# Jan-Celin/SCCG-genome-compression

Measured on AMD Instinct MI355X. Metric: target bases compressed/sec at 1/2/4/8 GPUs; bit-exact record stream vs CPU ref, higher is better.
Workload: dtype u8

## Files before the change

sccg-genome-compression_amd/csrc/walk.hip:

```cpp
#include "internal.h"

#include <algorithm>
#include <chrono>
#include <map>
#include <mutex>
#include <cstdio>
#include <cstdlib>
#include <vector>

namespace {

constexpr int WPB = 4;
constexpr int WWPB = 4;
constexpr int WCAP = 256;
constexpr int32_t INVALID = INT32_MIN;
constexpr int32_t NEVER = INT32_MIN + 1;
constexpr int ANCHOR_K = 32;
constexpr int KEY_K = 15;
constexpr int KMAX = 32;
constexpr int KB_COUNT = 32;
constexpr int ANCHOR_STEP = 64;
constexpr int ANCHOR_LOAD = 1;
constexpr int ANCHOR_PROBE_BATCHES = 2;
constexpr uint32_t A_MULTI = 0xFFFFFFFFu;
constexpr int ANCHOR_RETRIES = 8;
constexpr int32_t ANCHOR_RETRY_STEP = 512;
constexpr int32_t FROZEN_MIN = 4096;
constexpr int FROZEN_MAX = 256;
constexpr int FROZEN_FIRST = 16;

enum ChunkKind : int32_t { KIND_SPEC = 0, KIND_FIX = 1, KIND_RESUME = 2 };
enum ChunkStatus : int32_t { ST_OK = 0, ST_ESC = 1, ST_CONV = 3, ST_DONE = 4 };
constexpr int32_t RESEED_GAP = 1024;
constexpr int32_t TRAP_P = 4096;
constexpr int RESPEC_AHEAD = 256;
constexpr int RESPEC_MAX_TRIGGERS = 64;
constexpr int32_t LONG_GAP = 4096;
constexpr int32_t CAND_CAP = 65536;
constexpr int CH_BAND = 512;
constexpr int CH_TBITS = CH_BAND <= 2048 ? 13 : 14;
constexpr int CH_GRID = 512;
constexpr int CH_HCAP = 4096;
constexpr int32_t CHAIN_MCAP = 1 << 22;
constexpr int CH_GENS_PER_SYNC = 4;
constexpr int FF_MIN_CHUNKS = 8;
constexpr int64_t CH_FF_SPAN = 32 * 1024;
constexpr int CH_MAX_GENS = 4096;
constexpr int MARCH_ROUNDS = 4;
constexpr int CHAIN_ROUND = 10;
constexpr int64_t CH_DENSE_HITS = 32768;
constexpr int CH_DENSE_N = 32;
constexpr int32_t CH_DENSE_SPAN = 8192;
constexpr int CH_HANDBACK_N = 64;

struct WalkPtrs {
    const uint8_t* R;
    const uint8_t* T;
    int32_t nR, nT, k, m, S, C, cap;
    int32_t kp;
    int32_t xlo, xhi;
    int32_t* bt[2];
    int32_t* bp[2];
    int32_t* bl[2];
    int32_t* cnt[2];
    int32_t* cur;
    int32_t* exitX;
    int32_t* exitP;
    int32_t* usedX;
    int32_t* usedP;
    int32_t* kind;
    int32_t* status;
    int32_t* escX;
    int32_t* escP;
    int32_t* escN;
    int32_t* escQ;
    int32_t* snapX;
    int32_t* snapP;
    int32_t* guess;
    int32_t* plist;
    int32_t* rlist;
    int32_t* clist;
    int32_t* newX;
    int32_t* newP;
    int32_t* conv;
    int32_t* changed;
    int32_t* walked;
    int32_t* lround;
    int32_t* seedq;
    int32_t* trapped;
    int32_t* frozen;
    int32_t* flist;
    int32_t* fy;
    int32_t* scal;
    int32_t* trig;
    int32_t* tflag;
    int32_t* fa_j;
    int32_t* fa_l;
    int32_t* fa_p;
    int32_t* hintY;
    int32_t* hintP;
    uint64_t* atab;
    uint32_t agen;
    int32_t adet;
    uint32_t* fbits;
    uint32_t* cbits;
    int32_t round;
    int32_t abits;
    const int64_t* dnR;
    int32_t astep;
    unsigned long long* fc;
    unsigned long long* fcb;
    int32_t* cand;
    uint8_t* kb;
    int64_t* flat_off;
    int32_t* ft;
    int32_t* fp;
    int32_t* fl;
    int64_t* tlen;
    int64_t* partial;
    int64_t* scal64;
    int64_t* lgap;
    int64_t* cprev;
    int64_t* ctext;
    int64_t lgap_cap;
    int32_t* chs;
    int32_t* chm_t;
    int32_t* chm_p;
    int32_t* chm_l;
    int32_t chm_cap;
    int32_t ch_settled;
    int32_t* chh_y;
    uint32_t* chh_k;
    int32_t* chh_n;
    int32_t* chh_tr;
    uint64_t* dbg;
    int32_t dbg_phases;
    int32_t dbg_round;
};

__device__ __forceinline__ int32_t chunk_lo(const WalkPtrs& A, int32_t j) { return A.xlo + j * A.S; }
__device__ __forceinline__ int32_t chunk_hi(const WalkPtrs& A, int32_t j) {
    const int32_t lo = A.xlo + j * A.S;
    return lo + A.S < A.xhi ? lo + A.S : A.xhi;
}

constexpr int WFBITS = 14;
constexpr int LBV = 2048;
constexpr int LBW = LBV / 256;
static_assert(LBW % 8 == 0, "whole 32-byte stretches per lane");
constexpr int LEAD = 128;
static_assert(LEAD % (4 * LBW) == 0, "the lead is whole lanes' stretches");
__device__ __forceinline__ uint32_t wf_h1(uint32_t key) { return slot_hash(key, WFBITS); }
__device__ __forceinline__ uint32_t wf_h2(uint32_t key) { return (key * 0x85EBCA77u) >> (32 - WFBITS); }
__device__ __forceinline__ uint32_t wf_h3(uint32_t key) { return (key * 0xC2B2AE3Du + 0x27D4EB2Fu) >> (32 - WFBITS); }
struct WalkLds {
    uint32_t wbits[1 << (WFBITS - 5)];
    __attribute__((aligned(16))) uint8_t rbuf[LBV + 64];
    __attribute__((aligned(16))) uint8_t tbuf[LBV + 64];
};
constexpr int32_t NO_BUF = INT32_MIN / 2;
struct BufPos {
    int32_t rb0 = NO_BUF, tb0 = NO_BUF;
    __device__ __forceinline__ bool has_r(int32_t a, int32_t n) const { return a >= rb0 && a + n <= rb0 + LBV; }
    __device__ __forceinline__ bool has_t(int32_t a, int32_t n) const { return a >= tb0 && a + n <= tb0 + LBV; }
};

__device__ __forceinline__ uint64_t pick_key(int32_t p, int32_t pme) {
    const int32_t d = p - pme;
    return ((uint64_t)(uint32_t)(d < 0 ? -d : d) << 32) | (uint32_t)p;
}

__device__ __forceinline__ bool bytes_eq(const uint8_t* a, const uint8_t* b, int k) {
    for (int i = 0; i < k; i++) if (a[i] != b[i]) return false;
    return true;
}

template <int ND>
__device__ __forceinline__ void loadw_lds(const uint8_t* lds, int32_t off, uint32_t (&o)[ND]) {
    const uint32_t* w = reinterpret_cast<const uint32_t*>(lds) + (off >> 2);
    const uint32_t sh = (uint32_t)(off & 3);
    uint32_t v[ND + 1];
#pragma unroll
    for (int i = 0; i <= ND; i++) v[i] = w[i];
#pragma unroll
    for (int i = 0; i < ND; i++) o[i] = __builtin_amdgcn_alignbyte(v[i + 1], v[i], sh);
}

template <int ND>
__device__ __forceinline__ void loadw_sel(bool in_lds, const uint8_t* lds, int32_t lds_off, const uint8_t* g,
                                          uint32_t (&o)[ND]) {
    if (in_lds) {
        loadw_lds<ND>(lds, lds_off, o);
    } else {
        loadw<ND>(g, o);
        asm volatile("" ::: "memory");
    }
}

template <int N>
__device__ __forceinline__ int first_diff(const uint32_t (&r)[N], const uint32_t (&t)[N]) {
    int pos = 4 * N;
#pragma unroll
    for (int i = N - 1; i >= 0; i--) {
        const uint32_t x = r[i] ^ t[i];
        if (x) pos = 4 * i + (__builtin_ctz(x) >> 3);
    }
    return pos;
}
__device__ __forceinline__ int first_diff32(const uint32_t (&r)[8], const uint32_t (&t)[8]) { return first_diff<8>(r, t); }

__device__ __forceinline__ void lds16(const uint8_t* lds, int32_t off, uint32_t (&o)[4]) {
    const int32_t a = off + 16 * lane_id();
    const uint2* p = reinterpret_cast<const uint2*>(lds + (a & ~7));
    const uint2 v0 = p[0], v1 = p[1], v2 = p[2];
    const uint32_t sh = (uint32_t)(off & 3);
    uint32_t w[5];
    if (off & 4) { w[0] = v0.y; w[1] = v1.x; w[2] = v1.y; w[3] = v2.x; w[4] = v2.y; }
    else { w[0] = v0.x; w[1] = v0.y; w[2] = v1.x; w[3] = v1.y; w[4] = v2.x; }
#pragma unroll
    for (int i = 0; i < 4; i++) o[i] = __builtin_amdgcn_alignbyte(w[i + 1], w[i], sh);
}

__device__ __forceinline__ int32_t lds_first_diff(const uint8_t* rbuf, int32_t ra, const uint8_t* tbuf, int32_t tb, int32_t n) {
    const int lane = lane_id();
    for (int32_t base = 0; base < n; base += 1024) {
        const int32_t lim = n - base - 16 * lane;
        int e = 16;
        if (lim > 0) {
            uint32_t r[4], t[4];
            lds16(rbuf, ra + base, r);
            lds16(tbuf, tb + base, t);
            e = first_diff<4>(r, t);
            if (e >= lim) e = 16;
        }
        const unsigned long long m = __ballot(e < 16);
        if (m) {
            const int l = first_lane(m);
            return base + 16 * l + lane_val(e, l);
        }
    }
    return n;
}

__device__ __forceinline__ int32_t wave_lce(const WalkPtrs& A, WalkLds& L, BufPos& B, int32_t a, int32_t b, int32_t maxlen) {
    const int lane = lane_id();
    if (maxlen <= 0) return 0;
    int32_t off = 0;
    if (a >= B.rb0 && b >= B.tb0 && a < B.rb0 + LBV && b < B.tb0 + LBV) {
        int32_t avail = B.rb0 + LBV - a < B.tb0 + LBV - b ? B.rb0 + LBV - a : B.tb0 + LBV - b;
        if (avail > maxlen) avail = maxlen;
        const int32_t e = lds_first_diff(L.rbuf, a - B.rb0, L.tbuf, b - B.tb0, avail);
        if (e < avail || avail >= maxlen) return e;
        off = avail;
    }
    while (off < maxlen) {
        const int32_t lead = (a + off >= LEAD && b + off >= LEAD) ? LEAD : 0;
        const int32_t sa = (a + off - lead) & ~15, sb = (b + off - lead) & ~15;
        static_assert(LBV == 2048, "two KiB of each per step");
        const uint4* gr = reinterpret_cast<const uint4*>(A.R + sa) + lane;
        const uint4* gt = reinterpret_cast<const uint4*>(A.T + sb) + lane;
        const uint4 r0 = gr[0], r1 = gr[64], t0 = gt[0], t1 = gt[64];
        wave_sync();
        {
            uint4* dr = reinterpret_cast<uint4*>(L.rbuf) + lane;
            uint4* dt = reinterpret_cast<uint4*>(L.tbuf) + lane;
            dr[0] = r0; dr[64] = r1;
            dt[0] = t0; dt[64] = t1;
        }
        wave_sync();
        B.rb0 = sa;
        B.tb0 = sb;
        const int32_t ra = a + off - sa, tb = b + off - sb;
        int32_t avail = LBV - (ra > tb ? ra : tb);
        if (avail > maxlen - off) avail = maxlen - off;
        const int32_t e = lds_first_diff(L.rbuf, ra, L.tbuf, tb, avail);
        if (e < avail) return off + e;
        off += avail;
    }
    return maxlen;
}


__device__ int32_t wave_lce_hbm(const uint8_t* __restrict__ R, int32_t a, const uint8_t* __restrict__ T, int32_t b,
                                int32_t maxlen) {
    const int lane = lane_id();
    for (int32_t off = 0; off < maxlen; off += 2048) {
        const int32_t my = off + 32 * lane;
        int32_t e = INT32_MAX;
        if (maxlen - my > 0) {
            uint32_t r[8], t[8];
            loadw<8>(R + a + my, r);
            loadw<8>(T + b + my, t);
            int pos = first_diff32(r, t);
            if (maxlen - my < 32 && pos > maxlen - my) pos = maxlen - my;
            if (pos < 32) e = my + pos;
        }
        const unsigned long long sm = __ballot(e != INT32_MAX);
        if (sm) {
            const int32_t m = lane_val(e, first_lane(sm));
            return m < maxlen ? m : maxlen;
        }
    }
    return maxlen > 0 ? maxlen : 0;
}

__device__ __forceinline__ int32_t ext_k(const WalkPtrs& A, WalkLds& L, BufPos& B, int32_t c, int32_t y) {
    const int32_t kp = A.kp;
    int32_t maxlen = A.nR - (c + kp);
    const int32_t mt = A.nT - (y + kp);
    if (mt < maxlen) maxlen = mt;
    const int32_t l = kp + wave_lce(A, L, B, c + kp, y + kp, maxlen);
    return l >= A.k ? l : 0;
}

constexpr uint32_t KEY_NONE = 0x40000000u;
struct RegWin {
    int32_t P, lo, n;
    uint32_t key[4];
    uint32_t vmask;
};

__device__ __forceinline__ void reg_window(const WalkPtrs& A, int32_t P, RegWin& W, const WalkLds* L = nullptr,
                                           const BufPos* B = nullptr) {
    const int lane = lane_id(), k = A.k;
    W.P = P;
    W.lo = P - A.m < 0 ? 0 : P - A.m;
    const int32_t hi = (P + A.m < A.nR - k) ? P + A.m : A.nR - k;
    W.n = hi - W.lo + 1;
    if (W.n < 0) W.n = 0;
    W.vmask = 0;
    W.key[0] = W.key[1] = W.key[2] = W.key[3] = KEY_NONE;
    const bool lds = L && B->has_r(W.lo, W.n + 20);
    const int i0 = 4 * lane;
    if (i0 >= W.n) return;
    uint32_t w[5];
    loadw_sel<5>(lds, lds ? L->rbuf : nullptr, lds ? W.lo - B->rb0 + i0 : 0, A.R + W.lo + i0, w);
    uint64_t code;
    uint32_t bad;
    pack_codes<5>(w, code, bad);
    const int kp = A.kp;
    const uint32_t MASK = (1u << (2 * kp)) - 1u, KM = (1u << kp) - 1u;
#pragma unroll
    for (int q = 0; q < 4; q++) {
        W.key[q] = (bad >> q) & KM ? exotic_key(A.R + W.lo + i0 + q, kp) : (uint32_t)(code >> (2 * q)) & MASK;
        if (i0 + q < W.n) W.vmask |= 1u << q;
        else W.key[q] = KEY_NONE;
    }
}

__device__ __forceinline__ uint32_t target_key_w(const WalkPtrs& A, int32_t y, const uint32_t (&w)[4]) {
    const int kp = A.kp;
    uint64_t code;
    uint32_t bad;
    pack_codes<4>(w, code, bad);
    return bad & ((1u << kp) - 1u) ? exotic_key(A.T + y, kp) : (uint32_t)code & ((1u << (2 * kp)) - 1u);
}

__device__ __forceinline__ uint32_t win_match(const WalkPtrs& A, const RegWin& W, uint32_t kk, int32_t y) {
    uint32_t m = 0;
#pragma unroll
    for (int q = 0; q < 4; q++)
        if (((W.vmask >> q) & 1u) && W.key[q] == kk) m |= 1u << q;
    if (m && kk >= KEY_EXOTIC) {
        const int32_t c0 = W.lo + 4 * lane_id();
        for (int q = 0; q < 4; q++)
            if (((m >> q) & 1u) && !bytes_eq(A.R + c0 + q, A.T + y, A.kp)) m &= ~(1u << q);
    }
    return m;
}

__device__ __forceinline__ bool win_any(const RegWin& W, uint32_t kk) {
    return (W.key[0] == kk) | (W.key[1] == kk) | (W.key[2] == kk) | (W.key[3] == kk);
}

__device__ void bloom_window(const RegWin& W, WalkLds& L) {
    const int lane = lane_id();
    uint4* b4 = reinterpret_cast<uint4*>(L.wbits);
    for (int i = lane; i < (1 << (WFBITS - 5)) / 4; i += 64) b4[i] = make_uint4(0, 0, 0, 0);
    wave_sync();
#pragma unroll
    for (int q = 0; q < 4; q++) {
        if ((W.vmask >> q) & 1u) {
            const uint32_t f1 = wf_h1(W.key[q]), f2 = wf_h2(W.key[q]), f3 = wf_h3(W.key[q]);
            atomicOr(&L.wbits[f1 >> 5], 1u << (f1 & 31));
            atomicOr(&L.wbits[f2 >> 5], 1u << (f2 & 31));
            atomicOr(&L.wbits[f3 >> 5], 1u << (f3 & 31));
        }
    }
    wave_sync();
}

constexpr int WIDE = 16;
constexpr int WIDE_DEPTH = 1;
__device__ __forceinline__ int32_t wide_step(const WalkPtrs& A, const WalkLds& L, const RegWin& W, int32_t base, int32_t end,
                                             const uint32_t (&w)[8]) {
    const int lane = lane_id(), k = A.kp;
    const uint32_t MASK = (1u << (2 * k)) - 1u, KM = (1u << k) - 1u;
    const int32_t p0 = base + WIDE * lane;
    uint64_t code;
    uint32_t bad;
    pack_codes<8>(w, code, bad);
    uint32_t cand = 0;
#pragma unroll
    for (int st = 0; st < WIDE; st++) {
        const uint32_t key = (bad >> st) & KM ? KEY_EXOTIC : (uint32_t)(code >> (2 * st)) & MASK;
        const uint32_t f1 = wf_h1(key), f2 = wf_h2(key), f3 = wf_h3(key);
        if (key == KEY_EXOTIC ||
            ((L.wbits[f1 >> 5] >> (f1 & 31)) & (L.wbits[f2 >> 5] >> (f2 & 31)) & (L.wbits[f3 >> 5] >> (f3 & 31)) & 1u))
            cand |= 1u << st;
    }
    const int32_t lim = end - p0;
    if (lim < WIDE) cand &= lim > 0 ? (1u << lim) - 1u : 0u;
    for (unsigned long long hm = __ballot(cand != 0); hm; hm &= hm - 1) {
        const int l = __ffsll((long long)hm) - 1;
        uint32_t c = lane_val(cand, l);
        const uint32_t clo = lane_val((uint32_t)code, l), chi = lane_val((uint32_t)(code >> 32), l);
        const uint32_t cbad = lane_val(bad, l);
        const uint64_t lc = ((uint64_t)chi << 32) | clo;
        while (c) {
            const int st = __ffs((int)c) - 1;
            c &= c - 1;
            const int32_t y = base + WIDE * l + st;
            const uint32_t key = (cbad >> st) & KM ? exotic_key(A.T + y, k) : (uint32_t)(lc >> (2 * st)) & MASK;
            if (__ballot(win_match(A, W, key, y) != 0)) return y;
        }
    }
    return -1;
}

__device__ __forceinline__ int32_t wide_scan(const WalkPtrs& A, const WalkLds& L, const RegWin& W, int32_t x, int32_t end) {
    const int lane = lane_id();
    uint32_t w[WIDE_DEPTH][8];
#pragma unroll
    for (int d = 0; d < WIDE_DEPTH; d++)
        if (x + 64 * WIDE * d < end) loadw<8>(A.T + x + 64 * WIDE * d + WIDE * lane, w[d]);
    for (int32_t base = x; base < end;) {
#pragma unroll
        for (int d = 0; d < WIDE_DEPTH; d++) {
            uint32_t cur[8];
#pragma unroll
            for (int i = 0; i < 8; i++) cur[i] = w[d][i];
            const int32_t nb = base + 64 * WIDE * WIDE_DEPTH;
            if (nb < end) loadw<8>(A.T + nb + WIDE * lane, w[d]);
            const int32_t y = wide_step(A, L, W, base, end, cur);
            if (y >= 0) return y;
            base += 64 * WIDE;
            if (base >= end) return end;
        }
    }
    return end;
}

__device__ int32_t anchor_diag(const WalkPtrs& A, int32_t y0);
__device__ __forceinline__ int32_t anchor_diag_f(int32_t nT, const uint8_t* __restrict__ T, const uint64_t* __restrict__ atab, int32_t abits,
                                 uint32_t agen, int32_t y0);
#define ANCHOR_DIAG_KC(y) anchor_diag_f(KC->nT, KC->T, KC->atab, KC->abits, KC->agen, (y))

typedef const __attribute__((address_space(4))) WalkPtrs* KArgPtr;
__device__ __forceinline__ KArgPtr kargs() {
    KArgPtr p = (KArgPtr)(__builtin_amdgcn_kernarg_segment_ptr());
    asm volatile("" : "+s"(p));
    return p;
}
#define KC (kargs())

constexpr int DBG_SLOTS = 16;
constexpr int WALK_WAVES_PER_EU = 5;
template <bool DBG, bool CARRY>
__global__ __launch_bounds__(64 * WWPB) __attribute__((amdgpu_waves_per_eu(WALK_WAVES_PER_EU)))
void k_walk(WalkPtrs A, const int32_t* __restrict__ list, int32_t nlist, const int32_t* __restrict__ nlist_dev) {
    __shared__ WalkLds lds_all[WWPB];
    const int w = wave_in_block(), lane = lane_id();
    const int32_t li = (int32_t)blockIdx.x * WWPB + w;
    if (nlist_dev) nlist = *nlist_dev;
    if (CARRY && nlist > A.C) nlist = A.C;
    if (!CARRY && blockIdx.x == 0 && threadIdx.x == 0 && !KC->scal[9]) KC->scal[5] = 0;
    if (li >= nlist || KC->scal[9]) return;
    WalkLds& L = lds_all[w];
    int32_t j = uni(list[li]);
    const int32_t kind = CARRY ? KIND_FIX : uni(KC->kind[j]);
    int32_t lo_j = chunk_lo(A, j);
    int32_t hi_j = chunk_hi(A, j);
    const int32_t lastk = A.nT - A.k;

    int32_t x, P, n = 0, q = 0, ob, cb = -1, cc = 0;
    bool first_spec = false;
    if (CARRY) {
        cb = uni(KC->cur[j]);
        ob = 1 - cb;
        cc = uni(KC->cnt[cb][j]);
        x = uni(KC->newX[j - 1]);
        P = uni(KC->newP[j - 1]);
    } else if (kind == KIND_SPEC) {
        ob = uni(KC->cur[j]);
        x = lo_j;
        first_spec = uni(KC->usedX[j]) == NEVER;
        if (first_spec) {
            int32_t d = ANCHOR_DIAG_KC(lo_j);
            for (int i = 1; d == INVALID && i <= ANCHOR_RETRIES && lo_j + i * ANCHOR_RETRY_STEP < hi_j; i++)
                d = uni(ANCHOR_DIAG_KC(lo_j + i * ANCHOR_RETRY_STEP));
            P = INVALID;
            if (d != INVALID) {
                int64_t gp = (int64_t)lo_j - 1 + d;
                P = (int32_t)(gp < 0 ? 0 : (gp > A.nR - 1 ? A.nR - 1 : gp));
            }
            P = uni(P);
            if (lane == 0) KC->guess[j] = P;
        } else {
            P = uni(KC->guess[j]);
        }
        if (lane == 0) { KC->usedX[j] = lo_j; KC->usedP[j] = P; }
    } else if (kind == KIND_FIX) {
        cb = uni(KC->cur[j]);
        ob = 1 - cb;
        cc = uni(KC->cnt[cb][j]);
        x = uni(KC->snapX[j]);
        P = uni(KC->snapP[j]);
    } else {
        cb = uni(KC->cur[j]);
        ob = 1 - cb;
        cc = uni(KC->cnt[cb][j]);
        x = uni(KC->escX[j]);
        P = uni(KC->escP[j]);
        n = uni(KC->escN[j]);
        q = uni(KC->escQ[j]);
    }
    if (!CARRY) {
        if (lane == 0) KC->status[j] = ST_OK;
    }
    int32_t x_entry = x, P_entry = P;
    const uint64_t dbg_t0 = DBG ? wall_clock64() : 0;
    uint64_t dbg_c[13] = {};
    uint64_t tq = dbg_t0;
    const bool phases = DBG && A.dbg_phases;
    auto tick = [&](int slot) {
        if (DBG && phases) { const uint64_t t = wall_clock64(); dbg_c[slot] += t - tq; tq = t; }
    };
    if (P == INVALID) {
        if (lane == 0) { KC->cnt[ob][j] = 0; KC->exitX[j] = INVALID; KC->exitP[j] = INVALID; }
        return;
    }
    const size_t cap = (size_t)A.cap;
#define W_OT (KC->bt[ob] + (size_t)j * cap)
#define W_OP (KC->bp[ob] + (size_t)j * cap)
#define W_OL (KC->bl[ob] + (size_t)j * cap)
#define W_CT (KC->bt[cb] + (size_t)j * cap)
#define W_CP (KC->bp[cb] + (size_t)j * cap)
#define W_CL (KC->bl[cb] + (size_t)j * cap)

    RegWin W;
    W.P = INVALID;
    int32_t bloomP = INVALID;
    BufPos B;
    int32_t lme = x;
    bool converged = false, escalated = false;
    int32_t scan_end = hi_j < lastk + 1 ? hi_j : lastk + 1;
    if (!CARRY && kind == KIND_FIX) {
        const int32_t hy = uni(KC->hintY[j]);
        if (hy > x && hy < scan_end && uni(KC->hintP[j]) == P) x = hy;
    }
    int32_t old_seedq = cb >= 0 ? uni(KC->seedq[j]) : 0;
    int32_t seed_x = x, seedq = 0;
    int32_t cq0 = -1, ctv = INT32_MAX, cpv = 0, clv = 0;
    auto load_prev = [&](int32_t from) {
        cq0 = from;
        const int32_t qi = from + lane;
        ctv = qi < cc ? W_CT[qi] : INT32_MAX;
        cpv = qi < cc ? W_CP[qi] : 0;
        clv = qi < cc ? W_CL[qi] : 0;
    };
    if (cb >= 0) load_prev(q);
    int32_t rb_n0 = n, rbt = 0, rbp = 0, rbl = 0;
    auto flush_recs = [&]() {
        if (lane < n - rb_n0) { W_OT[rb_n0 + lane] = rbt; W_OP[rb_n0 + lane] = rbp; W_OL[rb_n0 + lane] = rbl; }
        rb_n0 = n;
    };
    for (;;) {
    while (x < scan_end) {
        if (DBG) tick(9);
        const int32_t y_l = x + lane;
        const bool valid = y_l < scan_end;
        uint32_t tw[4];
        loadw_sel<4>(B.has_t(x, 64 + 16), L.tbuf, y_l - B.tb0, A.T + y_l, tw);
        if (W.P != P) { reg_window(A, P, W, &L, &B); if (DBG) dbg_c[3]++; }
        if (DBG) tick(6);
        if (W.n <= 0) { x = scan_end; break; }
        if (DBG) dbg_c[1]++;
        const uint32_t key_l = valid ? target_key_w(A, y_l, tw) : 0u;
        int hl = -1;
        const int nb = scan_end - x < 64 ? scan_end - x : 64;
        for (int yy = 0; yy < nb; yy++) {
            const uint32_t kk = lane_val(key_l, yy);
            if (__ballot(win_any(W, kk)) && (kk < KEY_EXOTIC || __ballot(win_match(A, W, kk, x + yy) != 0))) {
                hl = yy;
                break;
            }
        }
        if (hl < 0) {
            x = (x + 64 < scan_end) ? x + 64 : scan_end;
            if (x < scan_end) {
                int32_t wend = scan_end;
                if (first_spec) {
                    if (x - (lme > seed_x ? lme : seed_x) >= RESEED_GAP) {
                        seed_x = x;
                        const int32_t d = ANCHOR_DIAG_KC(x);
                        if (d != INVALID) {
                            int64_t np = (int64_t)x - 1 + d;
                            np = np < 0 ? 0 : (np > A.nR - 1 ? A.nR - 1 : np);
                            if ((int32_t)np != P) { P = (int32_t)np; seedq = n; continue; }
                        }
                    }
                    const int32_t cpt = (lme > seed_x ? lme : seed_x) + RESEED_GAP;
                    if (cpt < wend) wend = cpt;
                }
                if (DBG) tick(9);
                if (bloomP != P) { bloom_window(W, L); bloomP = P; }
                if (DBG) tick(10);
                const int32_t x0 = x;
                x = wide_scan(A, L, W, x, wend);
                if (DBG) { dbg_c[2]++; dbg_c[12] += x - x0; tick(11); }
            }
            continue;
        }
        const int32_t y = x + hl;
        const uint32_t key = lane_val(key_l, hl);
        if (DBG) tick(7);
        const uint32_t mine = win_match(A, W, key, y);
        int32_t bl = 0, bcnt = 0;
        bool bhas0 = false;
        uint64_t bkey = ~0ull;
        int ncand = 0;
        for (int qq = 0; qq < 4; qq++) {
            unsigned long long cm = __ballot((mine >> qq) & 1u);
            while (cm) {
                const int cl_ = __ffsll((long long)cm) - 1;
                cm &= cm - 1;
                const int32_t c = W.lo + 4 * cl_ + qq;
                const int32_t l = ext_k(A, L, B, c, y);
                ncand++;
                if (!l) continue;
                if (l > bl) { bl = l; bcnt = 1; bhas0 = (c == 0); bkey = c ? pick_key(c, P) : ~0ull; }
                else if (l == bl) {
                    bcnt++;
                    if (c == 0) bhas0 = true;
                    else { const uint64_t pk = pick_key(c, P); bkey = pk < bkey ? pk : bkey; }
                }
            }
        }
        if (!bcnt) {
            x = y + 1;
            continue;
        }
        uint64_t pk;
        if (bcnt >= 2 && bhas0) pk = bkey;
        else { const uint64_t k0 = bhas0 ? pick_key(0, P) : ~0ull; pk = k0 < bkey ? k0 : bkey; }
        const int32_t p = (int32_t)(uint32_t)pk;
        if (p == 0) {
            escalated = true;
            if (lane == 0 && !CARRY) {
                if (kind == KIND_SPEC) { KC->cnt[ob][j] = 0; KC->exitX[j] = INVALID; KC->exitP[j] = INVALID; KC->usedP[j] = INVALID; }
                else {
                    KC->status[j] = ST_ESC;
                    KC->escX[j] = y; KC->escP[j] = P; KC->escN[j] = n; KC->escQ[j] = q;
                    atomicAdd(&KC->scal[1], 1);
                }
            }
            break;
        }
        {
            const int slot = n - rb_n0;
            if (lane == slot) { rbt = y; rbp = p; rbl = bl; }
            n++;
            if (slot == 63) flush_recs();
        }
        if (DBG) { dbg_c[0]++; dbg_c[4] += ncand; dbg_c[5] += bl; tick(8); }
        if (cb >= 0) {
            for (;;) {
                if (q >= cq0 + 64) load_prev(q);
                const int32_t qi = cq0 + lane;
                const bool ge = qi >= q && (qi >= cc || ctv >= y);
                const unsigned long long gm = __ballot(ge);
                if (gm) { q = cq0 + first_lane(gm); break; }
                q = cq0 + 64;
            }
            const int ql = q - cq0;
            if (q < cc && q >= old_seedq && lane_val(ctv, ql) == y && lane_val(cpv, ql) == p && lane_val(clv, ql) == bl) {
                flush_recs();
                const int32_t rest = cc - q - 1;
                for (int i = lane; i < rest; i += 64) {
                    W_OT[n + i] = W_CT[q + 1 + i];
                    W_OP[n + i] = W_CP[q + 1 + i];
                    W_OL[n + i] = W_CL[q + 1 + i];
                }
                n += rest;
                rb_n0 = n;
                converged = true;
                break;
            }
        }
        lme = y + bl;
        P = p + bl - 1;
        x = y + bl;
    }
    flush_recs();
    if (escalated) return;
    const int32_t nx = converged ? uni(KC->exitX[j]) : x, np = converged ? uni(KC->exitP[j]) : P;
    const bool frozen_end = !converged && x == hi_j && x - lme >= FROZEN_MIN;
    const bool trapped = !converged && x - x_entry >= A.S / 2 && (P - P_entry < TRAP_P && P_entry - P < TRAP_P);
    const bool exit_changed = nx != uni(KC->exitX[j]) || np != uni(KC->exitP[j]);
    if (!CARRY) {
        if (DBG && lane == 0 && (A.dbg_round < 0 || A.dbg_round == A.round)) {
            tick(9);
            uint64_t* d = KC->dbg + (size_t)j * DBG_SLOTS;
            d[0] = wall_clock64() - dbg_t0;
            for (int i = 0; i < 13; i++) d[1 + i] = dbg_c[i];
            d[14] = (uint64_t)A.round;
            d[15] = dbg_t0;
        }
        if (lane == 0) {
            KC->cnt[ob][j] = n;
            if (cb < 0) {
                KC->exitX[j] = x; KC->exitP[j] = P;
                KC->seedq[j] = seedq;
            } else {
                KC->newX[j] = nx; KC->newP[j] = np;
                KC->conv[j] = converged;
                KC->changed[j] = exit_changed;
                KC->walked[j] = A.round;
                KC->frozen[j] = frozen_end;
                KC->trapped[j] = trapped;
            }
            KC->status[j] = converged ? ST_CONV : ST_DONE;
        }
        if (kind != KIND_FIX || (j > 0 && uni(KC->lround[j - 1]) == A.round)) return;
        if (converged || !exit_changed || frozen_end || trapped) return;
        const int32_t j1 = j + 1;
        if (j1 >= A.C || uni(KC->lround[j1]) == A.round || (j1 + 1 < A.C && uni(KC->lround[j1 + 1]) == A.round)) return;
        if (lane == 0) {
            const int32_t at = atomicAdd(&KC->scal[11], 1);
            if (at < A.C) KC->clist[at] = j1;
            atomicOr(&KC->cbits[j1 >> 5], 1u << (j1 & 31));
        }
        return;
    } else {
        if (frozen_end) return;
        if (lane == 0) {
            KC->cnt[ob][j] = n;
            KC->cur[j] = ob;
            KC->exitX[j] = nx; KC->exitP[j] = np;
            KC->usedX[j] = x_entry; KC->usedP[j] = P_entry;
            KC->seedq[j] = 0;
            KC->conv[j] = converged;
            KC->changed[j] = exit_changed;
            KC->walked[j] = A.round;
            KC->frozen[j] = 0;
            KC->trapped[j] = trapped;
        }
    }
    if (converged || !exit_changed || frozen_end || trapped) return;
    const int32_t j1 = j + 1;
    if (j1 >= A.C || uni(KC->lround[j1]) == A.round || (j1 + 1 < A.C && uni(KC->lround[j1 + 1]) == A.round)) return;
    j = j1;
    lo_j = chunk_lo(A, j);
    hi_j = chunk_hi(A, j);
    scan_end = hi_j < lastk + 1 ? hi_j : lastk + 1;
    cb = uni(KC->cur[j]);
    ob = 1 - cb;
    cc = uni(KC->cnt[cb][j]);
    old_seedq = uni(KC->seedq[j]);
    n = 0;
    q = 0;
    rb_n0 = 0;
    seedq = 0;
    converged = false;
    x_entry = x;
    P_entry = P;
    load_prev(0);
    }
}

#undef W_OT
#undef W_OP
#undef W_OL
#undef W_CT
#undef W_CP
#undef W_CL

constexpr int LS_T = 256;
__device__ __forceinline__ void sort_list_block(const WalkPtrs& A, int32_t* __restrict__ list, const int32_t* __restrict__ count,
                                                uint32_t* __restrict__ bits, int32_t* wsum);
__global__ __launch_bounds__(LS_T) void k_commit(WalkPtrs A, const int32_t* __restrict__ list, int32_t nlist,
                                                 const int32_t* __restrict__ nlist_dev) {
    __shared__ int32_t wsum[LS_T / 64 + 1];
    __shared__ int last;
    if (A.scal[9]) return;
    if (nlist_dev) nlist = *nlist_dev;
    if (blockIdx.x == 0 && threadIdx.x < FROZEN_MAX) A.fy[threadIdx.x] = INT32_MAX;
    if (blockIdx.x == 0 && threadIdx.x == 0) A.scal[11] = 0;
    for (int32_t i = (int32_t)(blockIdx.x * blockDim.x + threadIdx.x); i < nlist; i += (int32_t)(gridDim.x * blockDim.x)) {
        const int32_t j = list[i];
        if (A.kind[j] == KIND_SPEC || A.status[j] == ST_ESC) continue;
        const int32_t round = A.round;
        const bool pred_changed = j > 0 && A.walked[j - 1] == round && A.changed[j - 1];
        if (!(A.conv[j] || !pred_changed)) continue;
        A.cur[j] = 1 - A.cur[j];
        A.exitX[j] = A.newX[j];
        A.exitP[j] = A.newP[j];
        A.usedX[j] = A.snapX[j];
        A.usedP[j] = A.snapP[j];
        A.seedq[j] = 0;
        if (A.frozen[j]) {
            A.flist[atomicAdd(&A.scal[5], 1)] = j;
            atomicOr(&A.fbits[j >> 5], 1u << (j & 31));
        }
    }
    if (!grid_last_block(reinterpret_cast<unsigned int*>(A.scal + 14), &last)) return;
    sort_list_block(A, A.flist, A.scal + 5, A.fbits, wsum);
}

__device__ __forceinline__ void sort_list_block(const WalkPtrs& A, int32_t* __restrict__ list, const int32_t* __restrict__ count,
                                                uint32_t* __restrict__ bits, int32_t* wsum) {
    if (*count <= 0) return;
    const int32_t nw = (A.C + 31) >> 5;
    const int32_t per = (nw + LS_T - 1) / LS_T, w0 = (int32_t)threadIdx.x * per;
    const int32_t w1 = w0 + per < nw ? w0 + per : nw;
    int c = 0;
    for (int32_t w = w0; w < w1; w++) c += __popc(bits[w]);
    const int incl = wave_incl_add<int>(c);
    const int wv = (int)(threadIdx.x >> 6), lane = lane_id();
    if (lane == 63) wsum[wv] = incl;
    __syncthreads();
    if (threadIdx.x == 0) {
        int run = 0;
        for (int i = 0; i < LS_T / 64; i++) { const int x = wsum[i]; wsum[i] = run; run += x; }
    }
    __syncthreads();
    int at = wsum[wv] + incl - c;
    for (int32_t w = w0; w < w1; w++) {
        uint32_t b = bits[w];
        if (!b) continue;
        bits[w] = 0;
        for (; b; b &= b - 1) list[at++] = (w << 5) + __ffs((int)b) - 1;
    }
}
__global__ __launch_bounds__(LS_T) void k_list_sort(WalkPtrs A, int32_t* __restrict__ list, const int32_t* __restrict__ count,
                                                    uint32_t* __restrict__ bits) {
    __shared__ int32_t wsum[LS_T / 64 + 1];
    if (A.scal[9]) return;
    sort_list_block(A, list, count, bits, wsum);
}

constexpr unsigned FZ_GRID = 256;
constexpr int FZ_T = SCCG_BLOCK;
__global__ __launch_bounds__(SCCG_BLOCK) void k_frozen_scan(WalkPtrs A, int fbase) {
    __shared__ WalkLds lds_all[WPB];
    if (A.scal[9]) return;
    const int fi = (int)blockIdx.y, f = fbase + fi;
    if (f >= A.scal[5]) return;
    const int32_t j = A.flist[f];
    const int32_t x0 = A.exitX[j], P = A.exitP[j];
    WalkLds& L = lds_all[wave_in_block()];
    RegWin W;
    reg_window(A, P, W);
    if (W.n <= 0) return;
    bloom_window(W, L);
    const int32_t end = A.nT - A.k + 1 < A.xhi ? A.nT - A.k + 1 : A.xhi;
    const int64_t gw = (int64_t)blockIdx.x * WPB + wave_in_block(), G = (int64_t)gridDim.x * WPB;
    for (int64_t base = x0 + gw * 64 * WIDE; base < end; base += G * 64 * WIDE) {
        if (base >= (int64_t)__hip_atomic_load(&A.fy[fi], __ATOMIC_RELAXED, __HIP_MEMORY_SCOPE_AGENT)) return;
        const int32_t seg_end = base + 64 * WIDE < end ? (int32_t)(base + 64 * WIDE) : end;
        const int32_t y = wide_scan(A, L, W, (int32_t)base, seg_end);
        if (y < seg_end) {
            if (lane_id() == 0) atomicMin(&A.fy[fi], y);
            return;
        }
    }
}

__device__ __forceinline__ int32_t fill_last(const WalkPtrs& A, int32_t j, int32_t y) {
    const int32_t lastk1 = A.nT - A.k + 1;
    const int32_t cap = A.xhi < lastk1 ? A.xhi : lastk1;
    if (y >= cap) return A.C - 1;
    if (y < A.xlo) return j;
    const int32_t q = (y - A.xlo) / A.S - 1;
    return q < j ? j : (q > A.C - 1 ? A.C - 1 : q);
}
template <bool DEV>
__global__ void k_walk_init(WalkPtrs A, int32_t startX, int32_t startP) {
    if (DEV && blockIdx.x == 0 && threadIdx.x == 0) {
        const unsigned long long* r = A.fc + 4;
        if (r[8] != 2 && r[0] == 0 && r[4] > 0) {
            const uint64_t k0 = 1ull << 32;
            const uint64_t pk = (r[5] >= 2 && r[6]) ? r[7] : ((r[6] && k0 < r[7]) ? k0 : r[7]);
            startX = (int32_t)r[4];
            startP = (int32_t)(uint32_t)pk + (int32_t)r[4] - 1;
        } else {
            startX = A.nT - A.k + 1;
            startP = INVALID;
        }
    }
    if (blockIdx.x == 0 && threadIdx.x == 0) A.scal[9] = DEV && startP == INVALID ? 1 : 0;
    for (int32_t j = (int32_t)(blockIdx.x * blockDim.x + threadIdx.x); j < A.C; j += (int32_t)(gridDim.x * blockDim.x)) {
        A.cur[j] = 0;
        A.cnt[0][j] = 0;
        A.cnt[1][j] = 0;
        A.usedX[j] = NEVER;
        A.usedP[j] = NEVER;
        A.exitX[j] = INVALID;
        A.exitP[j] = INVALID;
        A.kind[j] = j ? KIND_SPEC : KIND_FIX;
        A.plist[j] = j;
        A.lround[j] = 1;
        A.seedq[j] = 0;
        A.trapped[j] = 0;
        A.tflag[j] = 0;
        A.hintY[j] = -1;
        A.walked[j] = 0;
        A.changed[j] = 0;
        A.conv[j] = 0;
        A.frozen[j] = 0;
    }
    for (int32_t w = (int32_t)(blockIdx.x * blockDim.x + threadIdx.x); w <= A.C / 32; w += (int32_t)(gridDim.x * blockDim.x)) {
        A.fbits[w] = 0;
        A.cbits[w] = 0;
    }
    if (blockIdx.x == 0 && threadIdx.x == 0) {
        A.scal[0] = 0; A.scal[1] = 0; A.scal[2] = startX; A.scal[3] = startP;
        A.scal[5] = 0;
        A.scal[11] = 0;
        A.scal[14] = 0; A.scal[15] = 0;
        A.snapX[0] = startX;
        A.snapP[0] = startP;
    }
}

__global__ void k_spec_rest(WalkPtrs A) {
    const int32_t next = A.round + 1;
    for (int32_t q = (int32_t)(blockIdx.x * blockDim.x + threadIdx.x); q < A.C; q += (int32_t)(gridDim.x * blockDim.x)) {
        if (A.usedX[q] != NEVER || A.lround[q] == next) continue;
        A.kind[q] = KIND_SPEC;
        A.lround[q] = next;
        A.plist[atomicAdd(&A.scal[0], 1)] = q;
    }
}

__global__ __launch_bounds__(FROZEN_MAX) void k_round_fill(WalkPtrs A, int fbase, int fcap) {
    if (A.scal[9]) return;
    __shared__ int32_t rj[FROZEN_MAX], ry[FROZEN_MAX], sj[FROZEN_MAX], sy[FROZEN_MAX];
    const int t = (int)threadIdx.x;
    int nf = fcap > 0 ? A.scal[5] - fbase : 0;
    if (nf > fcap) nf = fcap;
    if (nf < 0) nf = 0;
    int32_t j = 0, y = 0;
    if (t < nf) { j = A.flist[fbase + t]; y = A.fy[t]; rj[t] = j; ry[t] = y; }
    __syncthreads();
    if (t < nf) {
        int r = 0;
        for (int f = 0; f < nf; f++) r += rj[f] < j || (rj[f] == j && f < t);
        sj[r] = j;
        sy[r] = y;
    }
    __syncthreads();
    if (t == 0) {
        int na = 0;
        int32_t filled_to = -1;
        for (int r = 0; r < nf; r++) {
            const int32_t jr = sj[r];
            if (jr <= filled_to || jr + 1 >= A.C) continue;
            const int32_t last = fill_last(A, jr, sy[r]);
            if (last > jr) { A.fa_j[na] = jr; A.fa_l[na] = last; A.fa_p[na] = A.exitP[jr]; na++; }
            if (last + 1 < A.C && sy[r] != INT32_MAX) { A.hintY[last + 1] = sy[r]; A.hintP[last + 1] = A.exitP[jr]; }
            filled_to = last;
        }
        A.scal[13] = na;
        A.scal[0] = 0;
        A.scal[12] = 0;
    }
}

constexpr int RT_T = 256;
__global__ __launch_bounds__(RT_T) void k_round_close(WalkPtrs A) {
    if (A.scal[9]) return;
    __shared__ int32_t fj[FROZEN_MAX], fl[FROZEN_MAX], fp[FROZEN_MAX];
    __shared__ int32_t trig[RESPEC_MAX_TRIGGERS];
    __shared__ int32_t wsum[RT_T / 64 + 1];
    __shared__ int last;
    const int na = A.scal[13];
    for (int i = (int)threadIdx.x; i < na; i += RT_T) { fj[i] = A.fa_j[i]; fl[i] = A.fa_l[i]; fp[i] = A.fa_p[i]; }
    __syncthreads();
    const int32_t next = A.round + 1;
    const int32_t lastk1 = A.nT - A.k + 1;
    auto filled = [&](int32_t q, int32_t* P) -> bool {
        int lo = 0, hi = na;
        while (lo < hi) {
            const int mid = (lo + hi) >> 1;
            if (fj[mid] < q) lo = mid + 1; else hi = mid;
        }
        if (lo == 0 || q > fl[lo - 1]) return false;
        *P = fp[lo - 1];
        return true;
    };
    const int32_t j = (int32_t)(blockIdx.x * blockDim.x + threadIdx.x);
    if (j < A.C) {
        int32_t ux, up, P = 0;
        if (na && filled(j, &P)) {
            const int32_t lo_j = chunk_lo(A, j), hi_j = chunk_hi(A, j);
            ux = lo_j < lastk1 ? lo_j : lastk1;
            up = P;
            A.cnt[A.cur[j]][j] = 0;
            A.usedX[j] = ux;
            A.usedP[j] = up;
            A.exitX[j] = hi_j < lastk1 ? hi_j : lastk1;
            A.exitP[j] = P;
            A.changed[j] = 0;
            A.seedq[j] = 0;
            A.trapped[j] = 0;
        } else {
            ux = A.usedX[j];
            up = A.usedP[j];
        }
        int32_t ex, ep;
        bool pred_trapped = false;
        if (j == 0) {
            ex = A.scal[2];
            ep = A.scal[3];
        } else if (na && filled(j - 1, &P)) {
            const int32_t hi_p = chunk_hi(A, j - 1);
            ex = hi_p < lastk1 ? hi_p : lastk1;
            ep = P;
        } else {
            ex = A.exitX[j - 1];
            ep = A.exitP[j - 1];
            pred_trapped = A.trapped[j - 1] != 0;
        }
        const int32_t lr = A.lround[j];
        const bool pend = ex != INVALID && !(ex == ux && ep == up);
        if (!pend) {
            if (lr == next) A.lround[j] = A.round;
        } else {
            A.snapX[j] = ex;
            A.snapP[j] = ep;
            A.kind[j] = KIND_FIX;
            A.lround[j] = next;
            A.plist[atomicAdd(&A.scal[0], 1)] = j;
            const bool tr = pred_trapped && A.walked[j - 1] == A.round;
            A.tflag[j] = tr ? A.round : -1;
            if (tr) atomicAdd(&A.scal[12], 1);
        }
    }
    if (!grid_last_block(reinterpret_cast<unsigned int*>(A.scal + 15), &last)) return;

    const int ntrig = A.scal[12];
    if (!ntrig) return;
    {
        const int32_t per = (A.C + RT_T - 1) / RT_T, c0 = (int32_t)threadIdx.x * per;
        int cnt = 0;
        for (int32_t q = c0; q < c0 + per && q < A.C; q++) cnt += A.tflag[q] == A.round && A.lround[q] == next;
        const int incl = wave_incl_add<int>(cnt);
        const int w = (int)(threadIdx.x >> 6), lane = lane_id();
        if (lane == 63) wsum[w] = incl;
        __syncthreads();
        if (threadIdx.x == 0) {
            int run = 0;
            for (int i = 0; i < RT_T / 64; i++) { const int x = wsum[i]; wsum[i] = run; run += x; }
            wsum[RT_T / 64] = run;
        }
        __syncthreads();
        int at = wsum[w] + incl - cnt;
        for (int32_t q = c0; q < c0 + per && q < A.C && at < RESPEC_MAX_TRIGGERS; q++)
            if (A.tflag[q] == A.round && A.lround[q] == next) trig[at++] = q;
        __syncthreads();
    }
    const int nt = wsum[RT_T / 64] < RESPEC_MAX_TRIGGERS ? wsum[RT_T / 64] : RESPEC_MAX_TRIGGERS;
    const int w = (int)(threadIdx.x >> 6), nw = (int)(blockDim.x >> 6), lane = lane_id();
    for (int t = w; t < nt; t += nw) {
        const int32_t jt = trig[t], P = A.snapP[jt];
        for (int32_t q0 = jt + 1; q0 <= jt + RESPEC_AHEAD && q0 < A.C; q0 += 64) {
            const int32_t q = q0 + lane;
            const bool ok = q < A.C && q <= jt + RESPEC_AHEAD && A.lround[q] != next;
            const unsigned long long okm = __ballot(ok);
// ... 2082 lines not shown
```

Measured before the change: 188.9 billion.

## Compare LCE in registers with one aligned stream, and converge early on previous records

The long-match extension now aligns the lower of the two positions to 16 bytes. It loads the other stream with unaligned 16-byte loads and finds the first mismatch directly from the loaded registers instead of rescanning shared memory. The chunk walker also checks, on entry and on carry to the next chunk, whether the current position already matches a record from the previous round. If it does, it copies the remaining records and marks the chunk converged, skipping the rescan. This adds unaligned global loads and more convergence logic, which could affect bit-exactness if the meet condition is wrong.

```diff
diff --git a/sccg-genome-compression_amd/csrc/walk.hip b/sccg-genome-compression_amd/csrc/walk.hip
--- a/sccg-genome-compression_amd/csrc/walk.hip
+++ b/sccg-genome-compression_amd/csrc/walk.hip
@@ -242,6 +242,27 @@
     return n;
 }
 
+__device__ __forceinline__ uint4 load16u(const uint8_t* __restrict__ p) {
+    uint4 v;
+    __builtin_memcpy(&v, p, 16);
+    return v;
+}
+
+__device__ __forceinline__ int first_diff16_from(const uint4& r, const uint4& t, int32_t from) {
+    uint32_t x[4] = {r.x ^ t.x, r.y ^ t.y, r.z ^ t.z, r.w ^ t.w};
+#pragma unroll
+    for (int i = 0; i < 4; i++) {
+        const int32_t sh = from - 4 * i;
+        if (sh >= 4) x[i] = 0;
+        else if (sh > 0) x[i] &= ~0u << (8 * sh);
+    }
+    int pos = 16;
+#pragma unroll
+    for (int i = 3; i >= 0; i--)
+        if (x[i]) pos = 4 * i + (__builtin_ctz(x[i]) >> 3);
+    return pos;
+}
+
 __device__ __forceinline__ int32_t wave_lce(const WalkPtrs& A, WalkLds& L, BufPos& B, int32_t a, int32_t b, int32_t maxlen) {
     const int lane = lane_id();
     if (maxlen <= 0) return 0;
@@ -255,11 +276,20 @@
     }
     while (off < maxlen) {
         const int32_t lead = (a + off >= LEAD && b + off >= LEAD) ? LEAD : 0;
-        const int32_t sa = (a + off - lead) & ~15, sb = (b + off - lead) & ~15;
+        const int32_t lo_pos = (a < b ? a : b) + off - lead;
+        const int32_t st = lead + (lo_pos & 15);
+        const int32_t sa = a + off - st, sb = b + off - st;
         static_assert(LBV == 2048, "two KiB of each per step");
-        const uint4* gr = reinterpret_cast<const uint4*>(A.R + sa) + lane;
-        const uint4* gt = reinterpret_cast<const uint4*>(A.T + sb) + lane;
-        const uint4 r0 = gr[0], r1 = gr[64], t0 = gt[0], t1 = gt[64];
+        uint4 r0, r1, t0, t1;
+        if (a < b) {
+            const uint4* gr = reinterpret_cast<const uint4*>(A.R + sa) + lane;
+            r0 = gr[0]; r1 = gr[64];
+            t0 = load16u(A.T + sb + 16 * lane); t1 = load16u(A.T + sb + 1024 + 16 * lane);
+        } else {
+            const uint4* gt = reinterpret_cast<const uint4*>(A.T + sb) + lane;
+            t0 = gt[0]; t1 = gt[64];
+            r0 = load16u(A.R + sa + 16 * lane); r1 = load16u(A.R + sa + 1024 + 16 * lane);
+        }
         wave_sync();
         {
             uint4* dr = reinterpret_cast<uint4*>(L.rbuf) + lane;
@@ -270,11 +300,28 @@
         wave_sync();
         B.rb0 = sa;
         B.tb0 = sb;
-        const int32_t ra = a + off - sa, tb = b + off - sb;
-        int32_t avail = LBV - (ra > tb ? ra : tb);
+        int32_t avail = LBV - st;
         if (avail > maxlen - off) avail = maxlen - off;
-        const int32_t e = lds_first_diff(L.rbuf, ra, L.tbuf, tb, avail);
-        if (e < avail) return off + e;
+        static_assert(LEAD + 16 <= 1024, "the start lies in the first KiB");
+        const int32_t end = st + avail;
+        {
+            int e = first_diff16_from(r0, t0, st - 16 * lane);
+            if (16 * lane + e >= end) e = 16;
+            const unsigned long long m = __ballot(e < 16);
+            if (m) {
+                const int l = first_lane(m);
+                return off + 16 * l + lane_val(e, l) - st;
+            }
+        }
+        if (end > 1024) {
+            int e = first_diff16_from(r1, t1, 0);
+            if (1024 + 16 * lane + e >= end) e = 16;
+            const unsigned long long m = __ballot(e < 16);
+            if (m) {
+                const int l = first_lane(m);
+                return off + 1024 + 16 * l + lane_val(e, l) - st;
+            }
+        }
         off += avail;
     }
     return maxlen;
@@ -555,10 +602,6 @@
     int32_t lme = x;
     bool converged = false, escalated = false;
     int32_t scan_end = hi_j < lastk + 1 ? hi_j : lastk + 1;
-    if (!CARRY && kind == KIND_FIX) {
-        const int32_t hy = uni(KC->hintY[j]);
-        if (hy > x && hy < scan_end && uni(KC->hintP[j]) == P) x = hy;
-    }
     int32_t old_seedq = cb >= 0 ? uni(KC->seedq[j]) : 0;
     int32_t seed_x = x, seedq = 0;
     int32_t cq0 = -1, ctv = INT32_MAX, cpv = 0, clv = 0;
@@ -575,6 +618,35 @@
         if (lane < n - rb_n0) { W_OT[rb_n0 + lane] = rbt; W_OP[rb_n0 + lane] = rbp; W_OL[rb_n0 + lane] = rbl; }
         rb_n0 = n;
     };
+    auto meet_prev = [&]() -> bool {
+        for (;;) {
+            const int32_t qi = cq0 + lane;
+            const unsigned long long hm = __ballot(qi < cc && qi >= old_seedq && ctv + clv == x && cpv + clv - 1 == P);
+            if (hm) {
+                const int32_t i1 = cq0 + first_lane(hm) + 1;
+                n = cc - i1;
+                for (int i = lane; i < n; i += 64) {
+                    W_OT[i] = W_CT[i1 + i];
+                    W_OP[i] = W_CP[i1 + i];
+                    W_OL[i] = W_CL[i1 + i];
+                }
+                rb_n0 = n;
+                converged = true;
+                x = scan_end;
+                return true;
+            }
+            if (cq0 + 64 >= cc || lane_val(ctv, 63) >= x) break;
+            load_prev(cq0 + 64);
+        }
+        q = cq0;
+        return false;
+    };
+    if (CARRY || kind == KIND_FIX) {
+        if (!meet_prev() && !CARRY) {
+            const int32_t hy = uni(KC->hintY[j]);
+            if (hy > x && hy < scan_end && uni(KC->hintP[j]) == P) x = hy;
+        }
+    }
     for (;;) {
     while (x < scan_end) {
         if (DBG) tick(9);
@@ -776,6 +848,7 @@
     x_entry = x;
     P_entry = P;
     load_prev(0);
+    meet_prev();
     }
 }
 
```

Result: no change. 191.8 billion, median of 6 (+1.5%).
